# OthmanB/TAMCMC-C

Measured on AMD Instinct MI355X. Metric: MCMC samples/sec (whole node), 1e5 nu-bins x 100 params x 20 tempered chains, higher is better.
Workload: dtype f64

## Files before the change

include/tamcmc_sampler.h:

```cpp
#ifndef TAMCMC_SAMPLER_H
#define TAMCMC_SAMPLER_H

#include <stdint.h>

#include "tamcmc_hip.h"

#ifdef __cplusplus
extern "C" {
#endif

typedef struct tamcmc_sampler tamcmc_sampler;

typedef struct tamcmc_sampler_config {
    int32_t model_id;
    int32_t prior_class;
    int32_t likelihood_id;
    int32_t use_drift;
    double likelihood_params;
    int64_t Nparams;
    const double *inputs;
    const int32_t *relax;
    const int32_t *plength;
    const double *priors;
    const int32_t *priors_switch;
// ... 17 lines not shown
void tamcmc_sampler_destroy(tamcmc_sampler *s);
int64_t tamcmc_sampler_nvars(const tamcmc_sampler *s);

#define TAMCMC_INFO_ENGINE 0
#define TAMCMC_INFO_NVARS 1
#define TAMCMC_INFO_NPARAMS 2
#define TAMCMC_INFO_NCHAINS 3
#define TAMCMC_INFO_ADAPT_IN_LDS 4
#define TAMCMC_INFO_FUSED_AVAILABLE 5
#define TAMCMC_INFO_CHAIN_GROUPS 6
#define TAMCMC_INFO_ITER_FUSED 7
#define TAMCMC_INFO_ITER_LOCKSTEP 8
#define TAMCMC_INFO_FUSED_STRETCHES 9
#define TAMCMC_INFO_QUICK_FALLBACKS 10
#define TAMCMC_INFO_QUICK_SURE 11
#define TAMCMC_SAMPLER_INFO_N 12
int tamcmc_sampler_get_info(const tamcmc_sampler *s, int64_t *info, int32_t n);

int tamcmc_sampler_run(tamcmc_sampler *s, int64_t n_iter, double *samples, double *stats);
int tamcmc_sampler_run_packed(tamcmc_sampler *const *s, int32_t S, int64_t n_iter, double *const *samples, double *const *stats);

int tamcmc_sampler_draws(const tamcmc_sampler *s, int64_t iteration, double *z, double *u_accept, double *u_swap, int32_t *ind_A);

int tamcmc_sampler_get_state(const tamcmc_sampler *s, double *vars, double *logL, double *logPrior, double *logPost,
                             double *Pmove, double *sigma, int64_t *counters);
int tamcmc_sampler_get_gradient(const tamcmc_sampler *s, double *grad, double *grad_prior, int32_t *valid);
int tamcmc_sampler_get_last_test(const tamcmc_sampler *s, double *vars_prop, double *stats_prop, double *lq, double *grad_prop);
int tamcmc_sampler_get_move_counts(const tamcmc_sampler *s, int64_t *moves);
int tamcmc_sampler_get_proposal(const tamcmc_sampler *s, int32_t m, double *mu, double *covarmat);
int tamcmc_sampler_set_proposal(tamcmc_sampler *s, int32_t m, const double *mu, const double *covarmat, double sigma);
int tamcmc_sampler_set_state(tamcmc_sampler *s, const double *vars, int64_t iteration);
// ... 33 lines not shown
```

tamcmc-c_amd/csrc/dev_sampler.h:

```cpp
#pragma once
#include <stdint.h>

#include "../../include/tamcmc_hip.h"
#if defined(__HIPCC__)
#include "dev_unpack.h"
#endif

#define TAMCMC_MAX_CHAINS 64

namespace tamcmc {

#if defined(__HIPCC__)
struct DevSamplerArgs {
    ModelDesc desc;
    int C, Nv, ntiles, chol_in_lds;
#ifdef TAMCMC_PROBE
    int probe = 0;
#endif
    int swap_rule;
    long pl;
    long dN_mixing;
    uint64_t seed;
    double c0, epsilon1, epsi2, A1, target_acceptance;
    const int *index_to_relax;
// ... 36 lines not shown

  public:
    DevSampler();
    ~DevSampler();
    DevSampler(const DevSampler &) = delete;
    DevSampler &operator=(const DevSampler &) = delete;
    int init(tamcmc_hip_ctx *ctx, const DevSamplerInit &in);
    int upload_state(const double *vars, const double *params, const double *logL, const double *logPr,
                     const double *logPost, const double *init_logL);
    int upload_proposal(int m, const double *L_rowmajor, const double *cov, const double *mu, double sigma);
    int download_state(double *vars, double *params, double *logL, double *logPr, double *logPost, double *Pmove,
                       int *moved, long *counters, long *moves_per_chain = nullptr);
    int download_proposal(int m, double *cov, double *mu, double *sigma);
    int download_gradient(double *grad, double *grad_prior);
    int download_last_proposal(double *vars_prop, double *grad_prop);
    void info(long out[11]) const;
    int run(long it0, long n_iter, const char *learn, double *samples, double *stats);
    int run_mala(long it0, long n_iter, const char *learn, double *samples, double *stats);
};

}
```

tamcmc-c_amd/csrc/dev_sampler.hip:

```cpp
#include <hip/hip_runtime.h>

#include <atomic>
#include <chrono>
#include <hip/hip_ext.h>

#include <cmath>
#include <cstdio>
#include <cstdlib>
#include <cstring>
#include <algorithm>
#include <type_traits>
#include <utility>
#include <vector>

#include "ctx.h"
#include "rgb_prestep.h"
#include "dev_sampler.h"
#include "kernels.h"
#include "loglike_tile.h"
#include "dev_unpack.h"
#include "fd_batch.h"
#include "mode_tables.h"
#include "rng.h"

// ... 647 lines not shown
    int xsplit;
    double *cand_vars, *cand_params;
    double *cand_logPr;
    int *cand_rej;
    int *cand_stP, *cand_stR;
    tamcmc_multiplet *mults;
    int *pairs, *nh, *nn;
    double *noise;
    double *bg;
    int *slot;
    double *prop_logPr;
    int *prop_st;
    double *quick;
    double *part;
    double *lz;
    double qmargin;
    unsigned long long *qcount;
};

constexpr int QN = 8;
constexpr int ST_L = 1, ST_BR = 2, ST_ENTRY = 4, ST_LZ = 8, ST_FIRST = 16, ST_COMMIT = 32;

typedef DevSamplerArgs __attribute__((address_space(4))) ConstArgs;
typedef FusedArgs __attribute__((address_space(4))) ConstFused;
__device__ __forceinline__ const void __attribute__((address_space(4))) *uniform_ptr(const void *p) {
    const unsigned long long v = (unsigned long long)p;
    const unsigned lo = (unsigned)__builtin_amdgcn_readfirstlane((int)(v & 0xffffffffull)), hi = (unsigned)__builtin_amdgcn_readfirstlane((int)(v >> 32));
    return (const void __attribute__((address_space(4))) *)(((unsigned long long)hi << 32) | lo);
}

struct Decided {
    int slot;
    int src;
    int src_acc;
    int src_par;
// ... 68 lines not shown
        const int swapped = resolve_swap(a, A, u, o0, o1);
        d.swap_first = A; d.swapped = swapped; d.src_par = p;
        const int B = A + 1;
        if (swapped) {
            if (m == A) { d.slot = 2 * C + (A >= f.xsplit ? 4 : 0) + accB; d.src = B; d.src_acc = accB; d.src_ps = ps1; d.r = rB; d.o = o0; }
            else { d.slot = 2 * C + (B >= f.xsplit ? 4 : 0) + 2 + accA; d.src = A; d.src_acc = accA; d.src_ps = ps0; d.r = rA; d.o = o1; }
        } else {
            if (m == A) { d.slot = 2 * A + accA; d.src = A; d.src_acc = accA; d.src_ps = ps0; d.r = rA; d.o = o0; }
            else { d.slot = 2 * B + accB; d.src = B; d.src_acc = accB; d.src_ps = ps1; d.r = rB; d.o = o1; }
        }
    }
    if (out && lane == 0) *out = d;
    return d.slot;
}

__device__ __attribute__((noinline)) void commit_chain(const DevSamplerArgs *ga, const FusedArgs *gf, int m, long it, int q, int settled, long rec,
                                                       int tiles, Decided *dec) {
    const int slot = decide(ga, gf, m, it, q, settled, dec);
    __syncthreads();
    const ConstArgs &a = *(const ConstArgs *)uniform_ptr(ga);
    const ConstFused &f = *(const ConstFused *)uniform_ptr(gf);
    const int lane = threadIdx.x, C = a.C, Nv = a.Nv, Np = a.desc.Np;
    const Decided d = *dec;
    if (lane == 0) {
        const size_t gs = (size_t)(it % 3) * f.NS + slot;
        const int stP0 = f.cand_stP[2 * gs], stP1 = f.cand_stP[2 * gs + 1], stR = f.cand_stR[gs];
        const double lp = f.cand_rej[gs] ? -INFINITY : f.cand_logPr[2 * gs] + f.cand_logPr[2 * gs + 1];
        const int stm = stP0 != TAMCMC_OK ? stP0 : (stP1 != TAMCMC_OK ? stP1 : stR);
        f.prop_logPr[q * C + m] = lp;
        f.prop_st[q * C + m] = stm;
        double *w = f.quick + ((size_t)q * C + m) * QN;
        const double Tm = a.Tcoefs[m];
        double Sstar = 0, ok = -1;
        double u, u1;
        rng_uniform2(a.seed, RNG_ACCEPT, (uint32_t)m, (uint64_t)it, 0, u, u1);
        if (stm == TAMCMC_OK && !(lp == -INFINITY || isnan(lp))) {
            const double cur = settled ? a.logPost_cur[q * C + m] : d.o.logPost;
            Sstar = -((log(u) - lp + cur) * Tm) / (double)a.pl;
// ... 34 lines not shown
        if (m == 0 && d.src_acc) a.counters[1] += 1;
        a.counters[8 + m] += d.src_acc;
        if (m == 0) a.counters[0] = it;
        if (d.swap_first == m) {
            atomicAdd((unsigned long long *)&a.counters[2], 1ull);
            if (d.swapped) atomicAdd((unsigned long long *)&a.counters[3], 1ull);
        }
        if (a.stats && rec >= 0) {
            double *r = a.stats + ((size_t)rec * C + m) * 3;
            r[0] = d.o.logL; r[1] = d.o.logPr; r[2] = d.o.logPost;
        }
        if (tiles && d.swap_first < 0 && f.quick[((size_t)(q ^ 1) * C + m) * QN + 1] == 2.0) atomicAdd(f.qcount + 1, 1ull);
    }
}

__device__ __attribute__((noinline)) int quick_decide_leaf(const DevSamplerArgs *ga, const FusedArgs *gf, int m, int q, int pairA, Decided *out) {
    const ConstArgs &a = *(const ConstArgs *)uniform_ptr(ga);
    const ConstFused &f = *(const ConstFused *)uniform_ptr(gf);
    const int lane = threadIdx.x & 63, C = a.C;
    const int p = q ^ 1, n2 = 2 * a.ntiles;
    const bool in_pair = pairA >= 0 && (m == pairA || m == pairA + 1);
    const int j0 = in_pair ? pairA : m;
    const double *b0 = f.part + ((size_t)p * C + j0) * n2;
    const double *r0 = f.quick + ((size_t)p * C + j0) * QN;
    const double rec = (lane < (in_pair ? 2 * QN : QN)) ? r0[lane] : 0.0;
    double s0 = 0, a0 = 0, s1 = 0, a1 = 0;
    for (int t0 = 0; t0 < n2; t0 += 512) {
        double v[8], w[8];
#pragma unroll
        for (int k = 0; k < 8; k++) {
            const int t = t0 + k * 64 + lane;
            v[k] = t < n2 ? b0[t] : 0.0;
            w[k] = (in_pair && t < n2) ? b0[n2 + t] : 0.0;
        }
#pragma unroll
        for (int k = 0; k < 8; k++) { s0 += v[k]; a0 += fabs(v[k]); s1 += w[k]; a1 += fabs(w[k]); }
    }
#pragma unroll
    for (int off = 32; off >= 1; off >>= 1) { s0 += __shfl_xor(s0, off, 64); a0 += __shfl_xor(a0, off, 64); }
    if (in_pair) {
#pragma unroll
        for (int off = 32; off >= 1; off >>= 1) { s1 += __shfl_xor(s1, off, 64); a1 += __shfl_xor(a1, off, 64); }
    }
    const double St0 = __shfl(rec, 0, 64), ok0 = __shfl(rec, 1, 64);
    const int ps0 = (int)__shfl(rec, 7, 64);
    const double mg = f.qmargin;
    int acc0 = 0;
    if (ok0 == 2.0) { s0 = 0; a0 = 0; }
    else if (ok0 > 0 && fabs(s0 - St0) > mg * (a0 + fabs(St0))) acc0 = s0 < St0 ? 1 : 0;
    else return -1;
    Decided d;
    d.swap_first = -1; d.swapped = 0; d.src_par = p; d.r = 0;
    d.o.acc = 0; d.o.r = 0; d.o.logL = 0; d.o.logPr = 0; d.o.logPost = 0;
    if (!in_pair) { d.slot = 2 * m + acc0; d.src = m; d.src_acc = acc0; d.src_ps = ps0; }
    else {
        const double St1 = __shfl(rec, QN, 64), ok1 = __shfl(rec, QN + 1, 64);
        const int ps1 = (int)__shfl(rec, QN + 7, 64);
        int acc1 = 0;
// ... 7 lines not shown
        const int swapped = x > lus ? 1 : 0;
        const int A = pairA, B = pairA + 1;
        d.swap_first = A; d.swapped = swapped;
        if (swapped) {
            if (m == A) { d.slot = 2 * C + (A >= f.xsplit ? 4 : 0) + acc1; d.src = B; d.src_acc = acc1; d.src_ps = ps1; }
            else { d.slot = 2 * C + (B >= f.xsplit ? 4 : 0) + 2 + acc0; d.src = A; d.src_acc = acc0; d.src_ps = ps0; }
        } else {
            if (m == A) { d.slot = 2 * A + acc0; d.src = A; d.src_acc = acc0; d.src_ps = ps0; }
            else { d.slot = 2 * B + acc1; d.src = B; d.src_acc = acc1; d.src_ps = ps1; }
        }
    }
    if (out && lane == 0) *out = d;
    return d.slot;
}

__device__ __forceinline__ int quick_decide(const DevSamplerArgs *ga, const FusedArgs *gf, int m, long it, int q, int settled, int pairA,
                                            Decided *out) {
    if (settled) return decide(ga, gf, m, it, q, 1, out);
    const int s = quick_decide_leaf(ga, gf, m, q, pairA, out);
    return s >= 0 ? s : decide(ga, gf, m, it, q, 0, out);
}

__device__ __attribute__((noinline)) int decide_counted(const DevSamplerArgs *ga, const FusedArgs *gf, int m, long it, int q, int tile) {
    if (tile == 0 && (threadIdx.x & 63) == 0) atomicAdd(((const ConstFused *)uniform_ptr(gf))->qcount, 1ull);
    return decide(ga, gf, m, it, q, 0, nullptr);
}
__device__ __forceinline__ int quick_slot(const DevSamplerArgs *ga, const FusedArgs *gf, int m, long it, int q, int settled, int pairA, int tile) {
    if (settled) return decide(ga, gf, m, it, q, 1, nullptr);
    const int s = quick_decide_leaf(ga, gf, m, q, pairA, nullptr);
    return s >= 0 ? s : decide_counted(ga, gf, m, it, q, tile);
}

struct StepTiles {
    const DevSamplerArgs *ga;
    const FusedArgs *gf;
    long it;
    int q, first, settled, pairA;
    static constexpr bool coherent_partials = false;
    __device__ __forceinline__ int slot(const LoglikeArgs &, int b, int tile) const { return quick_slot(ga, gf, first + b, it, q, settled, pairA, tile); }
    __device__ __forceinline__ void operator()(int, int, int) const {}
};

__device__ __attribute__((noinline)) void role_prior(const DevSamplerArgs *ga, const FusedArgs *gf, size_t gs, int h, const double *s_vars,
                                                     const double *s_params, const UnpackLds *Up) {
    const DevSamplerArgs &a = *ga;
    const FusedArgs &f = *gf;
    const UnpackLds U = *Up;
    const int Nv = a.Nv, Np = a.desc.Np, tid = threadIdx.x;
    if (h == 0) {
        for (int i = tid; i < Nv; i += 64) f.cand_vars[gs * Nv + i] = s_vars[i];
        for (int i = tid; i < Np; i += 64) f.cand_params[gs * Np + i] = s_params[i];
    }
    int rej = 0;
#ifdef TAMCMC_PROBE
// ... 53 lines not shown

__device__ __attribute__((noinline)) void lz_normals(const DevSamplerArgs *ga, long itn, int m, double *s_z) {
    normals_into(*ga, m, itn, s_z);
}
__device__ __attribute__((noinline)) void lz_rows(const DevSamplerArgs *ga, const FusedArgs *gf, int q_dst, int m, const double *s_z) {
    Lz_rows_wave(*ga, m, s_z, gf->lz + ((size_t)q_dst * ga->C + m) * ga->Nv);
}
__device__ __forceinline__ void lz_block(const DevSamplerArgs *ga, const FusedArgs *gf, long itn, int q_dst, int m, unsigned char *lds) {
    double *s_z = (double *)lds;
    lz_normals(ga, itn, m, s_z);
    __syncthreads();
    lz_rows(ga, gf, q_dst, m, s_z);
}

__device__ void candidate_role(const DevSamplerArgs &a, const FusedArgs &f, const DevSamplerArgs *ga, const FusedArgs *gf, long itn, int q_src,
                               int q_dst, int slot, int role, bool entry, int settled, int pairA, unsigned char *lds, Decided *dec) {
    if (role > 6) return;
    const int C = a.C, Nv = a.Nv, Np = a.desc.Np, tid = threadIdx.x;
    const int e_dst = (int)(itn % 3);
    int m, src, on_prop;
    if (slot < 2 * C) { m = slot >> 1; src = m; on_prop = slot & 1; }
    else {
        if (entry || !is_swap_iter(a, itn - 1)) return;
        const int A = swap_first(a, itn - 1, nullptr), e = slot - 2 * C;
        m = (e < 2) ? A : A + 1;
        src = (e < 2) ? A + 1 : A;
        on_prop = e & 1;
        slot += (m >= f.xsplit) ? 4 : 0;
    }
    if (entry && on_prop) return;
    if (entry && role == 0 && tid == 0) f.slot[q_src * C + m] = 2 * m;
// ... 3 lines not shown
#define RSTAMP(k) pt[k] = (long)wall_clock64()
#else
#define RSTAMP(k)
#endif
    double *s_params = (double *)lds;
    double *s_vars = s_params + Np;
    double *s_z = s_vars + Nv;
    const UnpackLds U = carve_unpack_lds((unsigned char *)(s_z + Nv + 1));
    __shared__ UnpackLds s_U;
    if (tid == 0) s_U = U;
    const double *bv, *bp;
    if (entry) {
        bv = a.vars_cur + ((size_t)q_src * C + src) * Nv;
        bp = a.params_cur + ((size_t)q_src * C + src) * Np;
    } else {
        const int ps = quick_decide(ga, gf, src, itn - 1, q_src, settled, pairA, dec);
        __syncthreads();
        const Decided d = *dec;
        if (on_prop) {
            const size_t gp = (size_t)((itn - 1) % 3) * f.NS + ps;
            bv = f.cand_vars + gp * Nv;
            bp = f.cand_params + gp * Np;
        } else if (d.src_acc) {
            const size_t gp = (size_t)((itn - 2) % 3) * f.NS + d.src_ps;
            bv = f.cand_vars + gp * Nv;
            bp = f.cand_params + gp * Np;
        } else {
            bv = a.vars_cur + ((size_t)d.src_par * C + d.src) * Nv;
            bp = a.params_cur + ((size_t)d.src_par * C + d.src) * Np;
        }
    }
// ... 42 lines not shown
    else role_background(ga, gf, e_dst, slot, role, s_params, &s_U);
#ifdef TAMCMC_PROBE
    __syncthreads();
    RSTAMP(3);
    if (tid == 0 && slot == 2 && !entry && role < 4) {
        long *w = a.counters + 8 + C + 8 * role;
        w[0] += pt[1] - pt[0]; w[1] += pt[2] - pt[1]; w[2] += pt[3] - pt[2]; w[3] += 1;
    }
#endif
#undef RSTAMP
}

struct StepCtl {
    long it, rec, it_lz;
    int q, flags;
    int nbr, nlz;
    int n_lz_live, q_lz;
    int first, cnt;
    int extra;
    int pairA;
    const DevSamplerArgs *ga;
    const struct FusedArgs *gf;
};

#define TAMCMC_STEP_BODY                                                                                                      \
    __shared__ tile::TileLds<MODE, 64> lds;                                                                                  \
    __shared__ Decided s_dec;                                                                                                \
    const int id = (int)blockIdx.x;                                                                                          \
    const int settled = (c.flags & ST_FIRST) ? 1 : 0;                                                                        \
     \
    if (id < c.nbr + c.nlz) __builtin_amdgcn_s_setprio(3);                                                                   \
    if (id < c.nbr) {                                                                                                        \
        const int k = id >> 3, slot = k < 2 * c.cnt ? 2 * c.first + k : 2 * a.C + (k - 2 * c.cnt);  \
        if (k >= 2 * c.cnt && !c.extra) return;                                                                              \
        if (c.flags & ST_ENTRY) candidate_role(a, f, c.ga, c.gf, c.it, c.q, c.q, slot, id & 7, true, 1, -1, (unsigned char *)&lds, &s_dec);    \
        else if (c.flags & ST_BR)                                                                                            \
            candidate_role(a, f, c.ga, c.gf, c.it + 1, c.q, c.q ^ 1, slot, id & 7, false, settled, c.pairA, (unsigned char *)&lds, &s_dec); \
        return;                                                                                                              \
    }                                                                                                                        \
    if (id < c.nbr + c.nlz) {                                                                                                \
        const int e = id - c.nbr, k = e - (c.nlz - c.cnt);                                                                   \
        if (k >= 0 && (c.flags & ST_COMMIT)) commit_chain(c.ga, c.gf, c.first + k, c.it, c.q, settled, c.rec, c.flags & ST_L, &s_dec); \
        else if (e < c.n_lz_live)                                                                                            \
            lz_block(c.ga, c.gf, c.it_lz + e / c.cnt, (c.q_lz ^ (e / c.cnt)) & 1, c.first + e % c.cnt, (unsigned char *)&lds);  \
        return;                                                                                                              \
    }                                                                                                                        \
    if (c.flags & ST_L)                                                                                                      \
        tile::loglike_tile<MODE, 64, K, false, false>(la, id - c.nbr - c.nlz, lds, StepTiles{c.ga, c.gf, c.it, c.q, c.first, settled, c.pairA});
template <int MODE, int K>
__global__ void __launch_bounds__(64) __attribute__((amdgpu_waves_per_eu(3))) k_step(const DevSamplerArgs a, const FusedArgs f, const LoglikeArgs la,
                                                                                      const StepCtl c) {
    TAMCMC_STEP_BODY
}
template <int MODE, int K>
__global__ void __launch_bounds__(64) k_step_wide(const DevSamplerArgs a, const FusedArgs f, const LoglikeArgs la, const StepCtl c) {
    TAMCMC_STEP_BODY
}
#undef TAMCMC_STEP_BODY

template <int MODE>
bool launch_step_k(int K, int grid, hipStream_t st, const DevSamplerArgs &a, const FusedArgs &f, const LoglikeArgs &la, const StepCtl &c,
                   hipEvent_t ev0, hipEvent_t ev1) {
    if (K == 4) hipExtLaunchKernelGGL((k_step<MODE, 4>), dim3(grid), dim3(64), 0, st, ev0, ev1, 0, a, f, la, c);
// ... 244 lines not shown
        I.ev_made = true;
    }
    {
        FusedArgs &f = I.f;
        f.NS = 2 * in.C + 8;
        {
            const int h = (int)(((long)in.C * 1) / 2);
            f.xsplit = (I.G == 2 && h >= 3 && in.C - h >= 3) ? h : in.C;
        }
        const size_t NS = (size_t)f.NS;
        DCHK(I.dalloc(&f.cand_vars, 3 * NS * Nv)); DCHK(I.dalloc(&f.cand_params, 3 * NS * Np)); DCHK(I.dalloc(&f.cand_logPr, 6 * NS));
        DCHK(I.dalloc(&f.cand_stP, 6 * NS)); DCHK(I.dalloc(&f.cand_stR, 3 * NS)); DCHK(I.dalloc(&f.cand_rej, 3 * NS));
        DCHK(I.dalloc(&f.mults, 3 * NS * (size_t)a.desc.per + 1)); DCHK(I.dalloc(&f.pairs, 6 * NS)); DCHK(I.dalloc(&f.nh, 3 * NS)); DCHK(I.dalloc(&f.nn, 3 * NS));
        DCHK(I.dalloc(&f.noise, 3 * NS * (size_t)a.desc.stride));
        DCHK(I.dalloc(&f.slot, 2 * C)); DCHK(I.dalloc(&f.prop_logPr, 2 * C)); DCHK(I.dalloc(&f.prop_st, 2 * C)); DCHK(I.dalloc(&f.quick, 2 * C * QN)); DCHK(I.dalloc(&f.lz, 2 * C * Nv));
        DCHK(I.dalloc(&f.qcount, 2));
        DCHK(hipMemsetAsync(f.qcount, 0, 2 * sizeof(unsigned long long), st));
        f.qmargin = 1e-11;
        DCHK(hipMemsetAsync(f.nn, 0, 3 * NS * sizeof(int), st));
        DCHK(hipMemsetAsync(f.cand_stP, 0, 6 * NS * sizeof(int), st));
        DCHK(hipMemsetAsync(f.cand_rej, 0, 3 * NS * sizeof(int), st));
        DCHK(hipMemsetAsync(f.cand_stR, 0, 3 * NS * sizeof(int), st));
        f.part = nullptr;
        f.bg = nullptr;
        const size_t role_lds = (Np + 2 * Nv + 1) * sizeof(double) + unpack_lds_bytes() + 32;
        I.fused_ok = !I.rgb && role_lds <= sizeof(tile::TileLds<tile::M_FAST_DIRECT, 64>);
    }
    DCHK(hipStreamSynchronize(st));
    return TAMCMC_OK;
}

int DevSampler::download_gradient(double *grad, double *grad_prior) {
// ... 8 lines not shown
    return TAMCMC_OK;
}

int DevSampler::download_last_proposal(double *vars_prop, double *grad_prop) {
    Impl &I = *impl;
    tamcmc_hip_ctx *c = I.ctx;
    if (!I.use_drift) return TAMCMC_ERR_BAD_ARG;
    DCHK(hipSetDevice(c->device));
    const size_t n = (size_t)I.a.C * I.a.Nv;
    DCHK(hipStreamSynchronize(c->stream));
    if (vars_prop) DCHK(hipMemcpy(vars_prop, I.a.vars_prop, n * sizeof(double), hipMemcpyDeviceToHost));
    if (grad_prop) DCHK(hipMemcpy(grad_prop, I.mala.grad_prop, n * sizeof(double), hipMemcpyDeviceToHost));
    return TAMCMC_OK;
}

void DevSampler::info(long out[11]) const {
    const Impl &I = *impl;
    unsigned long long qc[2] = {0, 0};
    if (I.f.qcount && hipSetDevice(I.ctx->device) == hipSuccess) (void)hipMemcpy(qc, I.f.qcount, sizeof qc, hipMemcpyDeviceToHost);
    out[8] = I.n_stretch; out[9] = (long)qc[0]; out[10] = (long)qc[1];
    out[0] = I.a.Nv; out[1] = I.a.desc.Np;
    out[2] = I.use_drift ? I.mala_chol_lds : I.a.chol_in_lds;
    out[3] = (I.fused_ok && !I.use_drift) ? 1 : 0;
    out[4] = I.G; out[5] = I.it_fused; out[6] = I.it_lockstep; out[7] = I.a.C;
}

int DevSampler::upload_state(const double *vars, const double *params, const double *logL, const double *logPr,
                             const double *logPost, const double *init_logL) {
    Impl &I = *impl;
    I.armed_it = -1;
    I.grad_valid = false;
    tamcmc_hip_ctx *c = I.ctx;
    DevSamplerArgs &a = I.a;
    const size_t C = (size_t)a.C, Np = (size_t)a.desc.Np, Nv = (size_t)a.Nv;
    hipStream_t st = c->stream;
// ... 325 lines not shown
            std::memcpy(img.data() + n1, &f, sizeof(FusedArgs));
            if (!I.d_argcopy) DCHK(I.dalloc(&I.d_argcopy, n1 + n2));
            if (img != I.h_argcopy) {
                DCHK(hipMemcpyAsync(I.d_argcopy, img.data(), n1 + n2, hipMemcpyHostToDevice, st));
                DCHK(hipStreamSynchronize(st));
                I.h_argcopy = img;
                I.armed_it = -1;
            }
            sc.ga = (const DevSamplerArgs *)I.d_argcopy;
            sc.gf = (const FusedArgs *)(I.d_argcopy + n1);
        }
        sc.first = 0; sc.cnt = a.C; sc.extra = 1;
        bool st_has_work = ia > 0;
        if (!(I.armed_it == it0 + ia && I.armed_q == q)) {
            st_has_work = true;
            sc.it = it0 + ia; sc.rec = -1; sc.q = q; sc.flags = ST_LZ; sc.nbr = 0; sc.nlz = nlz2; sc.n_lz_live = 2 * a.C; sc.it_lz = it0 + ia; sc.q_lz = q;
            DCHK(launch_step(c->precision, c->K, nlz2, st, args, f, lf[0], sc));
            sc.flags = ST_ENTRY; sc.nbr = nbr; sc.nlz = 0; sc.n_lz_live = 0;
            DCHK(launch_step(c->precision, c->K, nbr, st, args, f, lf[0], sc));
        }
        const bool timed = c->timing && fused_ev.size() < 16;
        const int fe = I.n_ev - 1 - (int)fused_ev.size();
        const bool split_ok = f.xsplit < a.C && c->step_scheme != 2 && (c->step_scheme == 3 || (long)a.C * a.ntiles >= 2500);
        const bool split = split_ok;
        if (timed && !split) DCHK(hipEventRecord(I.ev[fe][0], st));
        const int first1 = f.xsplit;
        hipStream_t s1 = I.gst[1];
        long n_split = 0, next_sample = len >= 97 ? 48 : len / 2;
        bool s1_ahead = false, s1_must_wait = st_has_work;
        auto swap_pair_of = [&](long it) -> int {
            if (!(a.C >= 2 && a.dN_mixing > 0 && (it % a.dN_mixing == 0) && it != 0)) return -1;
            double u, u2;
            rng_uniform2(a.seed, RNG_SWAP, 0, (uint64_t)it, 0, u, u2);
            int A = (int)(u2 * (double)(a.C - 1));
            if (A > a.C - 2) A = a.C - 2;
            return A;
        };
        auto launch_group = [&](int first, int cnt, int A, long i, bool settled, hipStream_t stream, hipEvent_t e0 = nullptr, hipEvent_t e1 = nullptr) -> int {
            const bool owns_pair = A >= first && A + 1 < first + cnt;
            sc.it = it0 + i; sc.rec = ((samples || stats) && !settled) ? i - 1 : (long)-1; sc.q = q;
            sc.flags = ST_L | ST_BR | ST_LZ | ST_COMMIT | (settled ? ST_FIRST : 0);
#ifdef TAMCMC_PROBE
            if (const char *ep = getenv("TAMCMC_PROBE_STEP")) {
                const int pm = atoi(ep);
                if (pm & 1) sc.flags &= ~ST_BR;
                if (pm & 2) sc.flags &= ~ST_COMMIT;
                if (pm & 4) sc.flags &= ~ST_LZ;
                if (pm & 8) sc.flags |= ST_FIRST;
                if (pm & 16) sc.flags &= ~ST_L;
            }
#endif
            sc.first = first; sc.cnt = cnt; sc.extra = owns_pair ? 1 : 0; sc.pairA = settled ? -1 : swap_pair_of(it0 + i - 1);
            sc.nbr = 8 * (2 * cnt + (owns_pair ? 4 : 0)); sc.nlz = ((2 * cnt + 7) / 8) * 8; sc.n_lz_live = cnt; sc.it_lz = it0 + i + 2; sc.q_lz = q;
            LoglikeArgs lq = lf[(it0 + i) % 3];
            lq.B = cnt;
            lq.partials = f.part + ((size_t)q * a.C + first) * a.ntiles * 2;
            DCHK(launch_step(c->precision, c->K, sc.nbr + sc.nlz + ntiles_pad * cnt, stream, args, f, lq, sc, e0, e1));
            return TAMCMC_OK;
        };
        auto launch_close = [&](int first, int cnt, hipStream_t stream) -> int {
            sc.it = it0 + ib; sc.rec = (samples || stats) ? ib - 1 : (long)-1; sc.q = q;
            sc.flags = ST_COMMIT;
            sc.first = first; sc.cnt = cnt; sc.extra = 0;
            sc.nbr = 0; sc.nlz = ((cnt + 7) / 8) * 8; sc.n_lz_live = 0; sc.it_lz = 0; sc.q_lz = 0;
            DCHK(launch_step(c->precision, c->K, sc.nlz, stream, args, f, lf[0], sc));
            return TAMCMC_OK;
        };
        auto straddles = [&](int A) { return split_ok && A == first1 - 1; };
        for (long i = ia; i < ib; i++) {
            const int A = swap_pair_of(it0 + i);
            const bool settled = i == ia;
            const bool joint = !split_ok || straddles(A) || (!settled && straddles(swap_pair_of(it0 + i - 1)));
            if (!joint) {
                if (s1_must_wait) {
                    DCHK(hipEventRecord(I.ev_fork, st));
                    DCHK(hipStreamWaitEvent(s1, I.ev_fork, 0));
                    s1_must_wait = false;
                }
// ... 231 lines not shown
```

tamcmc-c_amd/csrc/host_capi.cpp:

```cpp
#include <cmath>
#include <cstring>
#include <memory>
#include <vector>
#include <string>
#include <thread>

#include "../../include/tamcmc_sampler.h"
#include "dev_sampler.h"
#include "host_sampler.h"
#include "rng.h"

using namespace tamcmc;

extern "C" {
void tamcmc_hip_ctx_attach(tamcmc_hip_ctx *c);
void tamcmc_hip_ctx_detach(tamcmc_hip_ctx *c);
}

struct tamcmc_sampler {
    Config cfg;
    std::unique_ptr<MALA> mala;
    std::unique_ptr<Model_def> cur, prop;
    std::unique_ptr<DevSampler> dev;
    long accepted0 = 0;
// ... 127 lines not shown
    delete s;
    tamcmc_hip_ctx_detach(ctx);
}

int64_t tamcmc_sampler_nvars(const tamcmc_sampler *s) { return s ? s->cur->get_Nvars() : -1; }

int tamcmc_sampler_get_info(const tamcmc_sampler *s, int64_t *info, int32_t n) {
    if (!s || !info || n < 1) return TAMCMC_ERR_BAD_ARG;
    int64_t v[TAMCMC_SAMPLER_INFO_N] = {0};
    v[TAMCMC_INFO_ENGINE] = s->dev ? 1 : 0;
    v[TAMCMC_INFO_NVARS] = s->cur->get_Nvars();
    v[TAMCMC_INFO_NPARAMS] = s->cur->get_Nparams();
    v[TAMCMC_INFO_NCHAINS] = s->cfg.MALA.Nchains;
    v[TAMCMC_INFO_ADAPT_IN_LDS] = -1;
    if (s->dev) {
        long d[11];
        s->dev->info(d);
        v[TAMCMC_INFO_ADAPT_IN_LDS] = d[2];
        v[TAMCMC_INFO_FUSED_AVAILABLE] = d[3];
        v[TAMCMC_INFO_CHAIN_GROUPS] = d[4];
        v[TAMCMC_INFO_ITER_FUSED] = d[5];
        v[TAMCMC_INFO_ITER_LOCKSTEP] = d[6];
        v[TAMCMC_INFO_FUSED_STRETCHES] = d[8];
        v[TAMCMC_INFO_QUICK_FALLBACKS] = d[9];
        v[TAMCMC_INFO_QUICK_SURE] = d[10];
    }
    for (int32_t i = 0; i < n && i < TAMCMC_SAMPLER_INFO_N; i++) info[i] = v[i];
    return TAMCMC_OK;
}

int tamcmc_sampler_run(tamcmc_sampler *s, int64_t n_iter, double *samples, double *stats) {
    if (!s || n_iter < 0) return TAMCMC_ERR_BAD_ARG;
    const long Nc = s->cfg.MALA.Nchains, Nv = s->cur->get_Nvars();
    if (s->dev) {
        const long it0 = s->mala->iteration;
        std::vector<char> learn((size_t)n_iter);
        bool any = false;
        for (int64_t i = 0; i < n_iter; i++) { learn[(size_t)i] = s->mala->learn_at(it0 + i) ? 1 : 0; any = any || learn[(size_t)i]; }
        int rc = s->dev->run(it0, (long)n_iter, any ? learn.data() : nullptr, samples, stats);
        if (rc) return rc;
// ... 252 lines not shown
```

tamcmc-c_amd/csrc/loglike_tile.h:

```cpp
#pragma once
#include <hip/hip_runtime.h>
#include <stdint.h>

#include "kernels.h"
#include "bg_series.h"

namespace tamcmc {
namespace tile {

constexpr int CHUNK = 64;

constexpr int F_FULL = 1;
constexpr int F_SAFE = 2;
constexpr int F_ASYM = 4;
constexpr int F_FAR = 8;

constexpr int M_STRICT = 0, M_FAST_DIRECT = 2, M_FAST = 1;

constexpr int NC = 16;
constexpr double RHO_MAX2 = 1.0 / 36.0;
constexpr double RHO_MAX2_ASYM = 1.0 / 64.0;
constexpr int NH = bg::NH;
constexpr int ROW = NC + 2;

// ... 164 lines not shown
template <int MODE, int WGS>
struct __attribute__((aligned(16))) TileLds {
    static constexpr bool FARFIELD = (MODE == M_FAST);
    static constexpr int LDS_BYTES = FARFIELD ? (WGS * ROW * 8 > CHUNK * (int)sizeof(LdsMult) ? WGS * ROW * 8 : CHUNK * (int)sizeof(LdsMult))
                                              : CHUNK * (int)sizeof(LdsMult);
    unsigned char buf[LDS_BYTES];
    double coef[NC];
    double part[WGS / 16][NC];
    double red[2 * (WGS / 64)];
    double lt[TAMCMC_MAX_HARVEY];
    double lto[TAMCMC_MAX_HARVEY];
    int n, nfar, anyfar;
    unsigned short slot[CHUNK * 7];
};

template <int MODE, int WGS, int K, bool WRITE_MODEL, bool DELTA, bool COH = false>
__device__ __forceinline__ void tile_compute(const LoglikeArgs &a, const int tile, const int b, const int sb, TileLds<MODE, WGS> &S, const int mbeg,
                                             const int mend, const int nh, const int nn) {
    constexpr bool FAST = (MODE != M_STRICT);
    static_assert(!DELTA || (FAST && !WRITE_MODEL), "DELTA launches are FAST-mode, logL-only");
    constexpr bool FARFIELD = (MODE == M_FAST);
    LdsMult *s_m = (LdsMult *)S.buf;
    double *s_rows = (double *)S.buf;
    int &s_n = S.n, &s_nfar = S.nfar, &s_anyfar = S.anyfar;
    unsigned short *s_slot = S.slot;
    double *s_coef = S.coef;
    double(*s_part)[NC] = S.part;
    double *s_red = S.red;
    double *s_lt = S.lt, *s_lto = S.lto;
    const int tid = threadIdx.x;
#ifdef TAMCMC_PROBE
#define KSTAMP(k) do { if (a.dbg && b == 0 && tile == a.ntiles / 2 && tid == 0) a.dbg[k] = (long)wall_clock64(); } while (0)
#define PROBE_SKIP(bit) (a.probe & (bit))
// ... 372 lines not shown
        }
    }
    __syncthreads();
    double out[2];
    block_reduce<2, WGS>(s, s_red, out);
    if (tid == 0) {
        double *p = a.partials + ((size_t)b * a.ntiles + tile) * 2;
        if (COH) {
            typedef double __attribute__((address_space(1))) *gdp_t;
            __hip_atomic_store((gdp_t)p, out[0], __ATOMIC_RELAXED, __HIP_MEMORY_SCOPE_AGENT);
            __hip_atomic_store((gdp_t)p + 1, out[1], __ATOMIC_RELAXED, __HIP_MEMORY_SCOPE_AGENT);
        } else {
            p[0] = out[0];
            p[1] = out[1];
        }
    }
    KSTAMP(6);
#ifdef TAMCMC_PROBE
    if (a.dbg && a.dbg[7] == 77 && tid == 0) {
        long *w = a.dbg + 8 + 2 * ((size_t)b * a.ntiles + tile);
        w[0] = wg_t0;
        w[1] = (long)wall_clock64();
    }
#endif
#undef KSTAMP
#undef PROBE_SKIP
}

struct NoTail {
    static constexpr bool coherent_partials = false;
    __device__ __forceinline__ int slot(const LoglikeArgs &, int b, int ) const { return b; }
    __device__ __forceinline__ void operator()(int , int , int ) const {}
};

template <int MODE, int WGS, int K, bool WRITE_MODEL, bool DELTA, class Tail>
__device__ __forceinline__ void loglike_tile(const LoglikeArgs &a, const int id, TileLds<MODE, WGS> &S, const Tail &tail) {
    const int xcd = id & 7;
    int j = id >> 3, b, tile;
    if (a.prio_b < 0) {
        b = j % a.B;
        tile = (j / a.B) * 8 + xcd;
    } else {
        const int lead = ((a.ntiles + 7) >> 3) * 2;
        if (j < lead) {
            b = a.prio_b + (j & 1);
            tile = (j >> 1) * 8 + xcd;
        } else {
            j -= lead;
            const int rest = a.B - 2, r = j % rest;
            b = r + (r >= a.prio_b ? 2 : 0);
            tile = (j / rest) * 8 + xcd;
        }
    }
    if (tile >= a.ntiles) return;
    tile += a.tile_rot;
    if (tile >= a.ntiles) tile -= a.ntiles;
    const int sb = tail.slot(a, b, tile);
    const int nn = a.nnoise[sb], nh = a.nharvey[sb];
    const int mend = a.offsets[2 * sb + 1];
    const int mbeg = a.per > 0 ? (a.slot0 + sb) * a.per : a.offsets[2 * sb];
    if (nn > 0)
        tile_compute<MODE, WGS, K, WRITE_MODEL, DELTA, Tail::coherent_partials>(a, tile, b, sb, S, mbeg, mend, nh, nn);
    tail(b, tile, sb);
}

}
}
```

tamcmc-c_amd/sampler.py:

```python
import ctypes as C

import numpy as np

from . import ABI, EXTRA_ABI, HipContext, TamcmcError, OK, lib, _dp, _ip, _vp, _f64, _i32, _p

_i64p = C.POINTER(C.c_int64)


class SamplerConfig(C.Structure):
    _fields_ = [("model_id", C.c_int32), ("prior_class", C.c_int32), ("likelihood_id", C.c_int32), ("use_drift", C.c_int32),
                ("likelihood_params", C.c_double), ("Nparams", C.c_int64), ("inputs", _dp), ("relax", _ip), ("plength", _ip),
                ("priors", _dp), ("priors_switch", _ip), ("extra_priors", _dp), ("n_extra", C.c_int32),
                ("Nchains", C.c_int32), ("lambda_temp", C.c_double), ("target_acceptance", C.c_double), ("c0", C.c_double),
                ("epsilon1", C.c_double), ("epsilon2", C.c_double), ("A1", C.c_double), ("delta", C.c_double),
                ("delta_x", C.c_double), ("Nt_learn", _i64p), ("periods_learn", _i64p), ("n_Nt_learn", C.c_int32),
                ("engine", C.c_int32), ("dN_mixing", C.c_int64), ("init_errors", _dp), ("seed", C.c_uint64),
                ("fd_step_rel", C.c_double), ("chain_groups", C.c_int32), ("swap_rule", C.c_int32)]


EXTRA_ABI += [
    ("tamcmc_sampler_create", C.c_int, [C.POINTER(_vp), _vp, C.POINTER(SamplerConfig)]),
    ("tamcmc_sampler_destroy", None, [_vp]),
    ("tamcmc_sampler_nvars", C.c_int64, [_vp]),
    ("tamcmc_sampler_get_info", C.c_int, [_vp, _i64p, C.c_int32]),
# ... 103 lines not shown
        if st != OK:
            raise TamcmcError(st, self._L.tamcmc_hip_last_error(self.ctx._h).decode())
        return smp, stt

    def state(self):
        nc, nv = self.nchains, self.nvars
        out = {"vars": np.zeros((nc, nv)), "logL": np.zeros(nc), "logPrior": np.zeros(nc), "logPost": np.zeros(nc),
               "Pmove": np.zeros(nc), "sigma": np.zeros(nc)}
        cnt = np.zeros(4, dtype=np.int64)
        self._L.tamcmc_sampler_get_state(self._h, _p(out["vars"]), _p(out["logL"]), _p(out["logPrior"]), _p(out["logPost"]),
                                         _p(out["Pmove"]), _p(out["sigma"]), _p(cnt, _i64p))
        out.update(iteration=int(cnt[0]), accepted0=int(cnt[1]), swap_attempts=int(cnt[2]), swaps=int(cnt[3]))
        return out

    def info(self):
        v = np.zeros(12, dtype=np.int64)
        rc = self._L.tamcmc_sampler_get_info(self._h, _p(v, _i64p), 12)
        if rc != OK:
            raise TamcmcError(rc, "tamcmc_sampler_get_info")
        keys = ("engine", "nvars", "nparams", "nchains", "adapt_in_lds", "fused_available", "chain_groups", "iter_fused", "iter_lockstep",
                "fused_stretches", "quick_fallbacks", "quick_sure")
        return dict(zip(keys, (int(x) for x in v)))

    def gradient(self):
        g, gp = np.zeros((self.nchains, self.nvars)), np.zeros((self.nchains, self.nvars))
        v = np.zeros(self.nchains, dtype=np.int32)
        rc = self._L.tamcmc_sampler_get_gradient(self._h, _p(g), _p(gp), _p(v, _ip))
        if rc != OK:
            raise TamcmcError(rc, "tamcmc_sampler_get_gradient")
        return g, gp, v

    def last_test(self):
        v, st, lq = np.zeros((self.nchains, self.nvars)), np.zeros((self.nchains, 3)), np.zeros((self.nchains, 2))
        g = np.zeros((self.nchains, self.nvars))
        rc = self._L.tamcmc_sampler_get_last_test(self._h, _p(v), _p(st), _p(lq), _p(g))
        if rc != OK:
# ... 170 lines not shown
```

Baseline: 47600.

## Accumulate quick-decide partial sums via atomics in tiles instead of rescanning partials

Each loglike tile now atomically adds its partial sum and absolute sum into a small per-chain, phase-rotated accumulator buffer (triple-buffered by iteration mod 3). quick_decide_leaf then reads 8 pre-reduced slots instead of scanning all 2*ntiles partials per chain. The aim is to cut the reduction work and memory traffic on the critical decide path. In exchange it adds f64 global atomics per tile, zeroing of the next phase buffer in commit, and an extra mismatch check in commit_chain that reruns quick_decide_leaf and counts disagreements, which adds its own cost.

```diff
diff --git a/include/tamcmc_sampler.h b/include/tamcmc_sampler.h
--- a/include/tamcmc_sampler.h
+++ b/include/tamcmc_sampler.h
@@ -55,7 +55,8 @@
 #define TAMCMC_INFO_FUSED_STRETCHES 9
 #define TAMCMC_INFO_QUICK_FALLBACKS 10
 #define TAMCMC_INFO_QUICK_SURE 11
-#define TAMCMC_SAMPLER_INFO_N 12
+#define TAMCMC_INFO_QUICK_MISMATCH 12
+#define TAMCMC_SAMPLER_INFO_N 13
 int tamcmc_sampler_get_info(const tamcmc_sampler *s, int64_t *info, int32_t n);
 
 int tamcmc_sampler_run(tamcmc_sampler *s, int64_t n_iter, double *samples, double *stats);
diff --git a/tamcmc-c_amd/csrc/dev_sampler.h b/tamcmc-c_amd/csrc/dev_sampler.h
--- a/tamcmc-c_amd/csrc/dev_sampler.h
+++ b/tamcmc-c_amd/csrc/dev_sampler.h
@@ -74,7 +74,7 @@
     int download_proposal(int m, double *cov, double *mu, double *sigma);
     int download_gradient(double *grad, double *grad_prior);
     int download_last_proposal(double *vars_prop, double *grad_prop);
-    void info(long out[11]) const;
+    void info(long out[12]) const;
     int run(long it0, long n_iter, const char *learn, double *samples, double *stats);
     int run_mala(long it0, long n_iter, const char *learn, double *samples, double *stats);
 };
diff --git a/tamcmc-c_amd/csrc/dev_sampler.hip b/tamcmc-c_amd/csrc/dev_sampler.hip
--- a/tamcmc-c_amd/csrc/dev_sampler.hip
+++ b/tamcmc-c_amd/csrc/dev_sampler.hip
@@ -685,11 +685,13 @@
     double *quick;
     double *part;
     double *lz;
+    double *qsum;
     double qmargin;
     unsigned long long *qcount;
 };
 
 constexpr int QN = 8;
+constexpr int QSL = 8, QSW = 8;
 constexpr int ST_L = 1, ST_BR = 2, ST_ENTRY = 4, ST_LZ = 8, ST_FIRST = 16, ST_COMMIT = 32;
 
 typedef DevSamplerArgs __attribute__((address_space(4))) ConstArgs;
@@ -788,14 +790,26 @@
     return d.slot;
 }
 
+__device__ __attribute__((noinline)) int quick_decide_leaf(const DevSamplerArgs *ga, const FusedArgs *gf, int m, int q, int rph, int pairA, Decided *out);
 __device__ __attribute__((noinline)) void commit_chain(const DevSamplerArgs *ga, const FusedArgs *gf, int m, long it, int q, int settled, long rec,
-                                                       int tiles, Decided *dec) {
+                                                       int tiles, int ph, int pairA, Decided *dec) {
     const int slot = decide(ga, gf, m, it, q, settled, dec);
     __syncthreads();
     const ConstArgs &a = *(const ConstArgs *)uniform_ptr(ga);
     const ConstFused &f = *(const ConstFused *)uniform_ptr(gf);
     const int lane = threadIdx.x, C = a.C, Nv = a.Nv, Np = a.desc.Np;
     const Decided d = *dec;
+    if (!settled) {
+        const int qs = quick_decide_leaf(ga, gf, m, q, ph == 0 ? 2 : ph - 1, pairA, nullptr);
+        if (lane == 0 && qs >= 0 && qs != slot) atomicAdd(f.qcount + 2, 1ull);
+    }
+    if (lane < 3 * QSL) {
+        const int k = lane / QSL, zp = ph == 2 ? 0 : ph + 1;
+        if (!tiles || k == zp) {
+            double *z = f.qsum + (((size_t)k * C + m) * QSL + lane % QSL) * QSW;
+            z[0] = 0.0; z[1] = 0.0;
+        }
+    }
     if (lane == 0) {
         const size_t gs = (size_t)(it % 3) * f.NS + slot;
         const int stP0 = f.cand_stP[2 * gs], stP1 = f.cand_stP[2 * gs + 1], stR = f.cand_stR[gs];
@@ -860,34 +874,23 @@
     }
 }
 
-__device__ __attribute__((noinline)) int quick_decide_leaf(const DevSamplerArgs *ga, const FusedArgs *gf, int m, int q, int pairA, Decided *out) {
+__device__ __attribute__((noinline)) int quick_decide_leaf(const DevSamplerArgs *ga, const FusedArgs *gf, int m, int q, int rph, int pairA, Decided *out) {
     const ConstArgs &a = *(const ConstArgs *)uniform_ptr(ga);
     const ConstFused &f = *(const ConstFused *)uniform_ptr(gf);
     const int lane = threadIdx.x & 63, C = a.C;
-    const int p = q ^ 1, n2 = 2 * a.ntiles;
+    const int p = q ^ 1;
     const bool in_pair = pairA >= 0 && (m == pairA || m == pairA + 1);
     const int j0 = in_pair ? pairA : m;
-    const double *b0 = f.part + ((size_t)p * C + j0) * n2;
     const double *r0 = f.quick + ((size_t)p * C + j0) * QN;
+    const double2 *z0 = (const double2 *)(f.qsum + ((size_t)rph * C + j0) * QSL * QSW);
     const double rec = (lane < (in_pair ? 2 * QN : QN)) ? r0[lane] : 0.0;
-    double s0 = 0, a0 = 0, s1 = 0, a1 = 0;
-    for (int t0 = 0; t0 < n2; t0 += 512) {
-        double v[8], w[8];
+    double2 sa = make_double2(0.0, 0.0);
+    if (lane < (in_pair ? 2 * QSL : QSL)) sa = z0[(size_t)lane * (QSW / 2)];
+    double s0 = sa.x, a0 = sa.y;
 #pragma unroll
-        for (int k = 0; k < 8; k++) {
-            const int t = t0 + k * 64 + lane;
-            v[k] = t < n2 ? b0[t] : 0.0;
-            w[k] = (in_pair && t < n2) ? b0[n2 + t] : 0.0;
-        }
-#pragma unroll
-        for (int k = 0; k < 8; k++) { s0 += v[k]; a0 += fabs(v[k]); s1 += w[k]; a1 += fabs(w[k]); }
-    }
-#pragma unroll
-    for (int off = 32; off >= 1; off >>= 1) { s0 += __shfl_xor(s0, off, 64); a0 += __shfl_xor(a0, off, 64); }
-    if (in_pair) {
-#pragma unroll
-        for (int off = 32; off >= 1; off >>= 1) { s1 += __shfl_xor(s1, off, 64); a1 += __shfl_xor(a1, off, 64); }
-    }
+    for (int off = QSL / 2; off >= 1; off >>= 1) { s0 += __shfl_xor(s0, off, 64); a0 += __shfl_xor(a0, off, 64); }
+    double s1 = __shfl(s0, QSL, 64), a1 = __shfl(a0, QSL, 64);
+    s0 = __shfl(s0, 0, 64); a0 = __shfl(a0, 0, 64);
     const double St0 = __shfl(rec, 0, 64), ok0 = __shfl(rec, 1, 64);
     const int ps0 = (int)__shfl(rec, 7, 64);
     const double mg = f.qmargin;
@@ -925,10 +928,10 @@
     return d.slot;
 }
 
-__device__ __forceinline__ int quick_decide(const DevSamplerArgs *ga, const FusedArgs *gf, int m, long it, int q, int settled, int pairA,
+__device__ __forceinline__ int quick_decide(const DevSamplerArgs *ga, const FusedArgs *gf, int m, long it, int q, int rph, int settled, int pairA,
                                             Decided *out) {
     if (settled) return decide(ga, gf, m, it, q, 1, out);
-    const int s = quick_decide_leaf(ga, gf, m, q, pairA, out);
+    const int s = quick_decide_leaf(ga, gf, m, q, rph, pairA, out);
     return s >= 0 ? s : decide(ga, gf, m, it, q, 0, out);
 }
 
@@ -936,9 +939,9 @@
     if (tile == 0 && (threadIdx.x & 63) == 0) atomicAdd(((const ConstFused *)uniform_ptr(gf))->qcount, 1ull);
     return decide(ga, gf, m, it, q, 0, nullptr);
 }
-__device__ __forceinline__ int quick_slot(const DevSamplerArgs *ga, const FusedArgs *gf, int m, long it, int q, int settled, int pairA, int tile) {
+__device__ __forceinline__ int quick_slot(const DevSamplerArgs *ga, const FusedArgs *gf, int m, long it, int q, int rph, int settled, int pairA, int tile) {
     if (settled) return decide(ga, gf, m, it, q, 1, nullptr);
-    const int s = quick_decide_leaf(ga, gf, m, q, pairA, nullptr);
+    const int s = quick_decide_leaf(ga, gf, m, q, rph, pairA, nullptr);
     return s >= 0 ? s : decide_counted(ga, gf, m, it, q, tile);
 }
 
@@ -947,8 +950,19 @@
     const FusedArgs *gf;
     long it;
     int q, first, settled, pairA;
+    int rph;
+    double *qs;
     static constexpr bool coherent_partials = false;
-    __device__ __forceinline__ int slot(const LoglikeArgs &, int b, int tile) const { return quick_slot(ga, gf, first + b, it, q, settled, pairA, tile); }
+    __device__ __forceinline__ int slot(const LoglikeArgs &, int b, int tile) const { return quick_slot(ga, gf, first + b, it, q, rph, settled, pairA, tile); }
+    __device__ __forceinline__ void sums(int b, double s0, double s1) const {
+#ifdef TAMCMC_PROBE
+        if (!qs) return;
+#endif
+        typedef double __attribute__((address_space(1))) *gdp_t;
+        gdp_t w = (gdp_t)(qs + (size_t)b * (QSL * QSW));
+        __builtin_amdgcn_global_atomic_fadd_f64(w, s0 + s1);
+        __builtin_amdgcn_global_atomic_fadd_f64(w + 1, fabs(s0) + fabs(s1));
+    }
     __device__ __forceinline__ void operator()(int, int, int) const {}
 };
 
@@ -1032,7 +1046,7 @@
 }
 
 __device__ void candidate_role(const DevSamplerArgs &a, const FusedArgs &f, const DevSamplerArgs *ga, const FusedArgs *gf, long itn, int q_src,
-                               int q_dst, int slot, int role, bool entry, int settled, int pairA, unsigned char *lds, Decided *dec) {
+                               int q_dst, int slot, int role, bool entry, int settled, int pairA, int rph, unsigned char *lds, Decided *dec) {
     if (role > 6) return;
     const int C = a.C, Nv = a.Nv, Np = a.desc.Np, tid = threadIdx.x;
     const int e_dst = (int)(itn % 3);
@@ -1066,7 +1080,7 @@
         bv = a.vars_cur + ((size_t)q_src * C + src) * Nv;
         bp = a.params_cur + ((size_t)q_src * C + src) * Np;
     } else {
-        const int ps = quick_decide(ga, gf, src, itn - 1, q_src, settled, pairA, dec);
+        const int ps = quick_decide(ga, gf, src, itn - 1, q_src, rph, settled, pairA, dec);
         __syncthreads();
         const Decided d = *dec;
         if (on_prop) {
@@ -1139,6 +1153,7 @@
 struct StepCtl {
     long it, rec, it_lz;
     int q, flags;
+    int ph;
     int nbr, nlz;
     int n_lz_live, q_lz;
     int first, cnt;
@@ -1148,30 +1163,38 @@
     const struct FusedArgs *gf;
 };
 
+__device__ __forceinline__ double *step_qsum(const DevSamplerArgs &a, const FusedArgs &f, const StepCtl &c, int id) {
+#ifdef TAMCMC_PROBE
+    if (a.probe & 0x1000) return nullptr;
+#endif
+    return f.qsum + ((((size_t)c.ph * a.C + c.first) * QSL) + (id & 7)) * QSW;
+}
+
 #define TAMCMC_STEP_BODY                                                                                                      \
     __shared__ tile::TileLds<MODE, 64> lds;                                                                                  \
     __shared__ Decided s_dec;                                                                                                \
     const int id = (int)blockIdx.x;                                                                                          \
     const int settled = (c.flags & ST_FIRST) ? 1 : 0;                                                                        \
+    const int rph = c.ph == 0 ? 2 : c.ph - 1;                                        \
      \
     if (id < c.nbr + c.nlz) __builtin_amdgcn_s_setprio(3);                                                                   \
     if (id < c.nbr) {                                                                                                        \
         const int k = id >> 3, slot = k < 2 * c.cnt ? 2 * c.first + k : 2 * a.C + (k - 2 * c.cnt);  \
         if (k >= 2 * c.cnt && !c.extra) return;                                                                              \
-        if (c.flags & ST_ENTRY) candidate_role(a, f, c.ga, c.gf, c.it, c.q, c.q, slot, id & 7, true, 1, -1, (unsigned char *)&lds, &s_dec);    \
+        if (c.flags & ST_ENTRY) candidate_role(a, f, c.ga, c.gf, c.it, c.q, c.q, slot, id & 7, true, 1, -1, 0, (unsigned char *)&lds, &s_dec);    \
         else if (c.flags & ST_BR)                                                                                            \
-            candidate_role(a, f, c.ga, c.gf, c.it + 1, c.q, c.q ^ 1, slot, id & 7, false, settled, c.pairA, (unsigned char *)&lds, &s_dec); \
+            candidate_role(a, f, c.ga, c.gf, c.it + 1, c.q, c.q ^ 1, slot, id & 7, false, settled, c.pairA, rph, (unsigned char *)&lds, &s_dec); \
         return;                                                                                                              \
     }                                                                                                                        \
     if (id < c.nbr + c.nlz) {                                                                                                \
         const int e = id - c.nbr, k = e - (c.nlz - c.cnt);                                                                   \
-        if (k >= 0 && (c.flags & ST_COMMIT)) commit_chain(c.ga, c.gf, c.first + k, c.it, c.q, settled, c.rec, c.flags & ST_L, &s_dec); \
+        if (k >= 0 && (c.flags & ST_COMMIT)) commit_chain(c.ga, c.gf, c.first + k, c.it, c.q, settled, c.rec, c.flags & ST_L, c.ph, c.pairA, &s_dec); \
         else if (e < c.n_lz_live)                                                                                            \
             lz_block(c.ga, c.gf, c.it_lz + e / c.cnt, (c.q_lz ^ (e / c.cnt)) & 1, c.first + e % c.cnt, (unsigned char *)&lds);  \
         return;                                                                                                              \
     }                                                                                                                        \
     if (c.flags & ST_L)                                                                                                      \
-        tile::loglike_tile<MODE, 64, K, false, false>(la, id - c.nbr - c.nlz, lds, StepTiles{c.ga, c.gf, c.it, c.q, c.first, settled, c.pairA});
+        tile::loglike_tile<MODE, 64, K, false, false>(la, id - c.nbr - c.nlz, lds, StepTiles{c.ga, c.gf, c.it, c.q, c.first, settled, c.pairA, rph, step_qsum(a, f, c, id)});
 template <int MODE, int K>
 __global__ void __launch_bounds__(64) __attribute__((amdgpu_waves_per_eu(3))) k_step(const DevSamplerArgs a, const FusedArgs f, const LoglikeArgs la,
                                                                                       const StepCtl c) {
@@ -1446,8 +1469,10 @@
         DCHK(I.dalloc(&f.mults, 3 * NS * (size_t)a.desc.per + 1)); DCHK(I.dalloc(&f.pairs, 6 * NS)); DCHK(I.dalloc(&f.nh, 3 * NS)); DCHK(I.dalloc(&f.nn, 3 * NS));
         DCHK(I.dalloc(&f.noise, 3 * NS * (size_t)a.desc.stride));
         DCHK(I.dalloc(&f.slot, 2 * C)); DCHK(I.dalloc(&f.prop_logPr, 2 * C)); DCHK(I.dalloc(&f.prop_st, 2 * C)); DCHK(I.dalloc(&f.quick, 2 * C * QN)); DCHK(I.dalloc(&f.lz, 2 * C * Nv));
-        DCHK(I.dalloc(&f.qcount, 2));
-        DCHK(hipMemsetAsync(f.qcount, 0, 2 * sizeof(unsigned long long), st));
+        DCHK(I.dalloc(&f.qcount, 3));
+        DCHK(hipMemsetAsync(f.qcount, 0, 3 * sizeof(unsigned long long), st));
+        DCHK(I.dalloc(&f.qsum, 3 * C * QSL * QSW));
+        DCHK(hipMemsetAsync(f.qsum, 0, 3 * C * QSL * QSW * sizeof(double), st));
         f.qmargin = 1e-11;
         DCHK(hipMemsetAsync(f.nn, 0, 3 * NS * sizeof(int), st));
         DCHK(hipMemsetAsync(f.cand_stP, 0, 6 * NS * sizeof(int), st));
@@ -1486,11 +1511,11 @@
     return TAMCMC_OK;
 }
 
-void DevSampler::info(long out[11]) const {
+void DevSampler::info(long out[12]) const {
     const Impl &I = *impl;
-    unsigned long long qc[2] = {0, 0};
+    unsigned long long qc[3] = {0, 0, 0};
     if (I.f.qcount && hipSetDevice(I.ctx->device) == hipSuccess) (void)hipMemcpy(qc, I.f.qcount, sizeof qc, hipMemcpyDeviceToHost);
-    out[8] = I.n_stretch; out[9] = (long)qc[0]; out[10] = (long)qc[1];
+    out[8] = I.n_stretch; out[9] = (long)qc[0]; out[10] = (long)qc[1]; out[11] = (long)qc[2];
     out[0] = I.a.Nv; out[1] = I.a.desc.Np;
     out[2] = I.use_drift ? I.mala_chol_lds : I.a.chol_in_lds;
     out[3] = (I.fused_ok && !I.use_drift) ? 1 : 0;
@@ -1846,7 +1871,7 @@
         bool st_has_work = ia > 0;
         if (!(I.armed_it == it0 + ia && I.armed_q == q)) {
             st_has_work = true;
-            sc.it = it0 + ia; sc.rec = -1; sc.q = q; sc.flags = ST_LZ; sc.nbr = 0; sc.nlz = nlz2; sc.n_lz_live = 2 * a.C; sc.it_lz = it0 + ia; sc.q_lz = q;
+            sc.it = it0 + ia; sc.ph = (int)(sc.it % 3); sc.rec = -1; sc.q = q; sc.flags = ST_LZ; sc.nbr = 0; sc.nlz = nlz2; sc.n_lz_live = 2 * a.C; sc.it_lz = it0 + ia; sc.q_lz = q;
             DCHK(launch_step(c->precision, c->K, nlz2, st, args, f, lf[0], sc));
             sc.flags = ST_ENTRY; sc.nbr = nbr; sc.nlz = 0; sc.n_lz_live = 0;
             DCHK(launch_step(c->precision, c->K, nbr, st, args, f, lf[0], sc));
@@ -1870,7 +1895,7 @@
         };
         auto launch_group = [&](int first, int cnt, int A, long i, bool settled, hipStream_t stream, hipEvent_t e0 = nullptr, hipEvent_t e1 = nullptr) -> int {
             const bool owns_pair = A >= first && A + 1 < first + cnt;
-            sc.it = it0 + i; sc.rec = ((samples || stats) && !settled) ? i - 1 : (long)-1; sc.q = q;
+            sc.it = it0 + i; sc.ph = (int)(sc.it % 3); sc.rec = ((samples || stats) && !settled) ? i - 1 : (long)-1; sc.q = q;
             sc.flags = ST_L | ST_BR | ST_LZ | ST_COMMIT | (settled ? ST_FIRST : 0);
 #ifdef TAMCMC_PROBE
             if (const char *ep = getenv("TAMCMC_PROBE_STEP")) {
@@ -1891,9 +1916,9 @@
             return TAMCMC_OK;
         };
         auto launch_close = [&](int first, int cnt, hipStream_t stream) -> int {
-            sc.it = it0 + ib; sc.rec = (samples || stats) ? ib - 1 : (long)-1; sc.q = q;
+            sc.it = it0 + ib; sc.ph = (int)(sc.it % 3); sc.rec = (samples || stats) ? ib - 1 : (long)-1; sc.q = q;
             sc.flags = ST_COMMIT;
-            sc.first = first; sc.cnt = cnt; sc.extra = 0;
+            sc.first = first; sc.cnt = cnt; sc.extra = 0; sc.pairA = swap_pair_of(it0 + ib - 1);
             sc.nbr = 0; sc.nlz = ((cnt + 7) / 8) * 8; sc.n_lz_live = 0; sc.it_lz = 0; sc.q_lz = 0;
             DCHK(launch_step(c->precision, c->K, sc.nlz, stream, args, f, lf[0], sc));
             return TAMCMC_OK;
diff --git a/tamcmc-c_amd/csrc/host_capi.cpp b/tamcmc-c_amd/csrc/host_capi.cpp
--- a/tamcmc-c_amd/csrc/host_capi.cpp
+++ b/tamcmc-c_amd/csrc/host_capi.cpp
@@ -165,7 +165,7 @@
     v[TAMCMC_INFO_NCHAINS] = s->cfg.MALA.Nchains;
     v[TAMCMC_INFO_ADAPT_IN_LDS] = -1;
     if (s->dev) {
-        long d[11];
+        long d[12];
         s->dev->info(d);
         v[TAMCMC_INFO_ADAPT_IN_LDS] = d[2];
         v[TAMCMC_INFO_FUSED_AVAILABLE] = d[3];
@@ -175,6 +175,7 @@
         v[TAMCMC_INFO_FUSED_STRETCHES] = d[8];
         v[TAMCMC_INFO_QUICK_FALLBACKS] = d[9];
         v[TAMCMC_INFO_QUICK_SURE] = d[10];
+        v[TAMCMC_INFO_QUICK_MISMATCH] = d[11];
     }
     for (int32_t i = 0; i < n && i < TAMCMC_SAMPLER_INFO_N; i++) info[i] = v[i];
     return TAMCMC_OK;
diff --git a/tamcmc-c_amd/csrc/loglike_tile.h b/tamcmc-c_amd/csrc/loglike_tile.h
--- a/tamcmc-c_amd/csrc/loglike_tile.h
+++ b/tamcmc-c_amd/csrc/loglike_tile.h
@@ -202,9 +202,10 @@
     unsigned short slot[CHUNK * 7];
 };
 
-template <int MODE, int WGS, int K, bool WRITE_MODEL, bool DELTA, bool COH = false>
+template <int MODE, int WGS, int K, bool WRITE_MODEL, bool DELTA, class Hook>
 __device__ __forceinline__ void tile_compute(const LoglikeArgs &a, const int tile, const int b, const int sb, TileLds<MODE, WGS> &S, const int mbeg,
-                                             const int mend, const int nh, const int nn) {
+                                             const int mend, const int nh, const int nn, const Hook &hook) {
+    constexpr bool COH = Hook::coherent_partials;
     constexpr bool FAST = (MODE != M_STRICT);
     static_assert(!DELTA || (FAST && !WRITE_MODEL), "DELTA launches are FAST-mode, logL-only");
     constexpr bool FARFIELD = (MODE == M_FAST);
@@ -607,6 +608,7 @@
             p[0] = out[0];
             p[1] = out[1];
         }
+        hook.sums(b, out[0], out[1]);
     }
     KSTAMP(6);
 #ifdef TAMCMC_PROBE
@@ -623,6 +625,7 @@
 struct NoTail {
     static constexpr bool coherent_partials = false;
     __device__ __forceinline__ int slot(const LoglikeArgs &, int b, int ) const { return b; }
+    __device__ __forceinline__ void sums(int , double, double) const {}
     __device__ __forceinline__ void operator()(int , int , int ) const {}
 };
 
@@ -653,7 +656,7 @@
     const int mend = a.offsets[2 * sb + 1];
     const int mbeg = a.per > 0 ? (a.slot0 + sb) * a.per : a.offsets[2 * sb];
     if (nn > 0)
-        tile_compute<MODE, WGS, K, WRITE_MODEL, DELTA, Tail::coherent_partials>(a, tile, b, sb, S, mbeg, mend, nh, nn);
+        tile_compute<MODE, WGS, K, WRITE_MODEL, DELTA>(a, tile, b, sb, S, mbeg, mend, nh, nn, tail);
     tail(b, tile, sb);
 }
 
diff --git a/tamcmc-c_amd/sampler.py b/tamcmc-c_amd/sampler.py
--- a/tamcmc-c_amd/sampler.py
+++ b/tamcmc-c_amd/sampler.py
@@ -141,12 +141,12 @@
         return out
 
     def info(self):
-        v = np.zeros(12, dtype=np.int64)
-        rc = self._L.tamcmc_sampler_get_info(self._h, _p(v, _i64p), 12)
+        v = np.zeros(13, dtype=np.int64)
+        rc = self._L.tamcmc_sampler_get_info(self._h, _p(v, _i64p), 13)
         if rc != OK:
             raise TamcmcError(rc, "tamcmc_sampler_get_info")
         keys = ("engine", "nvars", "nparams", "nchains", "adapt_in_lds", "fused_available", "chain_groups", "iter_fused", "iter_lockstep",
-                "fused_stretches", "quick_fallbacks", "quick_sure")
+                "fused_stretches", "quick_fallbacks", "quick_sure", "quick_mismatch")
         return dict(zip(keys, (int(x) for x in v)))
 
     def gradient(self):
```

Result: faster. 49080 (median of 6 runs) (+3.1%).
